# KlrShaK/opencv-SimpleSLAM

Measured on AMD Instinct MI355X. Metric: frames/sec ALIKED+LightGlue @1241x376, higher is better.
Workload: dtype f32 (contractions: f16 hi/lo split operands, f32 accumulate; 3 MFMA per product, 2 in attention's P.V = precision 'f16x3p1', the default since r05: profiles/r05_flip_soak.md, r06_flip_soak.md); 1 GPU; C2/C4: synthetic 1241x376x3 uint8 frame stream, ALIKED-n16 extract + LightGlue match (t-1,t), 2048 kpts/frame, min_conf 0.7, random-init weights; inputs resident in HBM before the timed region, features and matches left on the device (the `pcie` leg times the same pipeline with per-round H2D of the frames and D2H of {count, pairs}); max_kpts=2048, lightglue_layers_executed=9, pairs_per_lightglue_launch=8, frames_per_aliked_launch=8

## Files before the change

### opencv-simpleslam_amd/csrc/lg_plan.hpp

```cpp
#pragma once

namespace sslam {

constexpr int LG_NH = 4;
constexpr int LG_NL = 9;
constexpr int LG_AQ = 128;
constexpr int LG_AK = 64;

constexpr int lg_ks_max(int Kc) { return Kc >= 1024 ? 4 : (Kc >= 512 ? 2 : 1); }

struct LGHooks {
    int precision = 2;
    bool sim_exact = false;
    int layers = LG_NL;
    bool self_only = false;
    int key_split = 0;
    int big_gemm = -1;
    int study = 0;
    bool share_frames = true;
};

enum class LGAttn { F32, FourWave, Asm };
enum class LGMerge { None, Launch, InFfn };
enum class LGLinears { Ring, Big };
enum class LGFfnTile { T64, T32 };

struct LGPlan {
    bool split;
    bool proj_split;
    LGAttn attn;
    bool p_single;
    int ks;
    LGMerge merge;
    LGLinears linears;
    LGFfnTile ffn_tile;
    bool heads_in_ffn;
    int layers;
    bool self_only_last;
    bool share_frames;
};

inline LGPlan lg_plan(const LGHooks& h, int Kc, int NI, bool want_heads) {
    LGPlan p{};
    p.split = h.precision != 0;
    p.proj_split = p.split && !h.sim_exact;
    p.layers = h.layers;
    p.self_only_last = h.self_only;
    p.share_frames = h.share_frames && p.split;

    const int k = h.key_split;
    const bool forced = k > 0, by_size = k == 0 || k == -4 || k == -5;
    const bool asm_kernel = k == 0 || k == -3 || k == -5 || k > 100;
    const bool fold_allowed = k == 0 || k > 100;
    p.ks = forced ? (k > 100 ? k - 100 : k) : 1;
    if (by_size) {
        const int units = NI * LG_NH * (Kc / LG_AQ);
        while (p.ks < 4 && units * p.ks < 256 && Kc / LG_AK >= 2 * p.ks * 4) p.ks *= 2;
    }
    if (p.ks > lg_ks_max(Kc)) p.ks = lg_ks_max(Kc);

    if (!p.split) {
        p.attn = LGAttn::F32;
        p.merge = LGMerge::Launch;
        return p;
    }
    p.attn = asm_kernel && !(h.study & 0x04) ? LGAttn::Asm : LGAttn::FourWave;
    p.p_single = h.precision == 2 || (h.study & 0x04);

    const int b = h.big_gemm;
    const bool big = b >= 0 ? b != 0 : ((long)NI * Kc >= 4096 && Kc % 128 == 0);
    p.linears = big ? LGLinears::Big : LGLinears::Ring;
    p.ffn_tile = b == 3 || (b != 2 && NI * (Kc / 64) <= 128) ? LGFfnTile::T32 : LGFfnTile::T64;
    p.heads_in_ffn = big && b != 5 && want_heads;

    if (p.ks == 1) p.merge = LGMerge::None;
    else p.merge = big && p.ffn_tile == LGFfnTile::T32 && h.study == 0 && fold_allowed ? LGMerge::InFfn : LGMerge::Launch;
    return p;
}

template <class PX, class PD, class PC>
inline int lg_alias(int NI, const PX* xy, const PD* desc, const PC* cnt, const int* bound, const float* size_w,
                    const float* size_h, int* rep) {
    int distinct = 0;
    for (int j = 0; j < NI; ++j) {
        rep[j] = j;
        for (int i = 0; i < j; ++i)
            if (xy[i] == xy[j] && desc[i] == desc[j] && cnt[i] == cnt[j] && bound[i] == bound[j] && size_w[i] == size_w[j] &&
                size_h[i] == size_h[j]) {
                rep[j] = i;
                break;
            }
        distinct += rep[j] == j;
    }
    return distinct;
}

}
```

### opencv-simpleslam_amd/csrc/lightglue_kernels.hip

```cpp
#include <mutex>
#include <type_traits>
#include "common.hpp"
#include "gemm_f32.hpp"
#include "gemm_f16x3.hpp"
#include "gemm_f16x3_big.hpp"
#include "ffn_fused.hpp"
#include "lg_plan.hpp"

namespace {

using sslam::f32x16;
using sslam::mfma32;
using sslam::acc_row;
using sslam::GemmSmem;
using sslam::GemmA;
using sslam::gemm_mainloop;
using sslam::half8;
using sslam::half4;
using sslam::SplitPtr;
using sslam::GemmSmemH;
using sslam::GemmAH;
using sslam::gemm_mainloop_h;
using sslam::gemm_mainloop_ring;
using sslam::panel_index;
using sslam::mfma16;
using sslam::split_f32;
using sslam::SPLIT_INV;
using sslam::LGHooks; using sslam::LGPlan; using sslam::LGAttn; using sslam::LGMerge; using sslam::LGLinears; using sslam::LGFfnTile;

constexpr int D = 256;
constexpr int DH = 64;
constexpr int NH = sslam::LG_NH;
constexpr int DIN = 128;
constexpr int NL = sslam::LG_NL;
constexpr int ENC = 32;

struct LGCtrl {
    int n[2];
    int n_prev[2];
// ... 933 lines not shown
    const int img = blockIdx.y, r = p.al.rep[img];
    const LGCtrl& pc = ctrl_of(p.ctrl, img);
    if (pc.stop) return;
    if (blockIdx.x == 0 && threadIdx.x == 0 && *range_flag_of(p.shadow, r)) *range_flag_of(p.ctrl, img) = 1;
    if (r == img) return;
    const unsigned n = (unsigned)pc.n[img & 1];
    const unsigned t = blockIdx.x * blockDim.x + threadIdx.x, nt = gridDim.x * blockDim.x;
    auto copy_rows = [&](void* base, size_t per) {
        uint4* d = reinterpret_cast<uint4*>(base) + (size_t)img * p.Kc * per;
        const uint4* s = reinterpret_cast<const uint4*>(base) + (size_t)r * p.Kc * per;
        for (unsigned u = t; u < n * per; u += nt) d[u] = s[u];
    };
    copy_rows(p.x, D * 4 / 16);
    copy_rows(p.enc_cos, ENC * 4 / 16);
    copy_rows(p.enc_sin, ENC * 4 / 16);
    constexpr unsigned PU = sslam::PANEL_K * 2 / 16;
    const unsigned run = n * PU;
    uint4* hi = reinterpret_cast<uint4*>(p.xs_hi);
    uint4* lo = reinterpret_cast<uint4*>(p.xs_lo);
    for (unsigned u = t; u < run * (D / sslam::PANEL_K); u += nt) {
        const unsigned k = u / run, e = u - k * run;
        const size_t po = (size_t)k * p.rows_total * PU + e;
        const size_t di = po + (size_t)img * p.Kc * PU, si = po + (size_t)r * p.Kc * PU;
        hi[di] = hi[si];
        lo[di] = lo[si];
    }
}

enum { EPH_QKV = 0, EPH_CROSS = 1, EPH_SPLIT = 2, EPH_F32 = 3, EPH_RESID = 4 };

struct LinearArgsH {
    SplitPtr A0, A1; int lda; int K0; int K;
    SplitPtr W; const float* bias; int N;
    float* out; int ldo;
    SplitOut outs;
    SplitOut q, k, vt;
    float q_scale, k_scale;
    const float* enc_cos; const float* enc_sin;
    const LGCtrl* ctrl; int Kc; int NIc;
};

constexpr int RING_MAX = 2;
template <int BM, int BN>
constexpr int ring_depth() {
    constexpr int stage_bytes = sslam::ring_stage_halves<BM, BN>() * 2;
    constexpr int d = (160 * 1024) / stage_bytes;
    return d > RING_MAX ? RING_MAX : (d < 2 ? 2 : d);
}

__device__ __forceinline__ float erf_as(float x) {
    const float ax = fabsf(x);
    const float t = __builtin_amdgcn_rcpf(fmaf(0.3275911f, ax, 1.0f));
    float p = fmaf(t, 1.061405429f, -1.453152027f);
    p = fmaf(p, t, 1.421413741f);
    p = fmaf(p, t, -0.284496736f);
    p = fmaf(p, t, 0.254829592f);
    const float e = __builtin_amdgcn_exp2f(-ax * ax * 1.4426950408889634f);
    return copysignf(fmaf(-p * t, e, 1.0f), x);
}

template <int BM, int BN, int TM, int TN, int WN, int NT, int EPI>
__device__ __forceinline__ void linear_h_epilogue(const LinearArgsH& p, const RowDom& rd, int col0, size_t ibase,
                                                  const f32x16 (&c1)[TM][TN], const f32x16 (&c2)[TM][TN],
                                                  _Float16* lds) {
    const int t = threadIdx.x, lane = t & 63, wave = t >> 6;
    const int wm = wave / WN, wn = wave % WN;
// ... 136 lines not shown
    RowDom rd;
    rd.img = rb / nb; rd.row0 = (rb % nb) * BM; rd.n = n_of(p.ctrl, rd.img);
    if (ctrl_of(p.ctrl, rd.img).stop) return;
    if (rd.row0 >= rd.n) return;
    const int col0 = cb * BN;
    const size_t ibase = (size_t)rd.img * p.Kc;
    GemmAH ga{{p.A0.hi, p.A0.lo}, {p.A1.hi ? p.A1.hi : p.A0.hi, p.A1.lo ? p.A1.lo : p.A0.lo}, p.lda, p.K0};
    f32x16 c1[TM][TN], c2[TM][TN];
    gemm_mainloop_ring<BM, BN, TM, TN, ring_depth<BM, BN>()>(ga, p.W, p.NIc * p.Kc, p.K, (int)ibase + rd.row0,
                                                             (int)ibase + p.Kc, col0, p.N, lg_ring, c1, c2);
    if (threadIdx.x >= 256) return;
    linear_h_epilogue<BM, BN, TM, TN, 2, 256, EPI>(p, rd, col0, ibase, c1, c2, lg_ring);
}

template <int BM, int BN, int WM, int WN, int EPI>
__global__ __launch_bounds__(WM * WN * 64, 2) void lg_linear_big_kernel(LinearArgsH p) {
    extern __shared__ __attribute__((aligned(16))) _Float16 lg_ring[];
    constexpr int TM = BM / (32 * WM), TN = BN / (32 * WN);
    int rb, cb;
    xcd_tile(gridDim.x, rb, cb);
    const int nb = (p.Kc + BM - 1) / BM;
    RowDom rd;
    rd.img = rb / nb; rd.row0 = (rb % nb) * BM; rd.n = n_of(p.ctrl, rd.img);
    if (ctrl_of(p.ctrl, rd.img).stop) return;
    if (rd.row0 >= rd.n) return;
    const int col0 = cb * BN;
    const size_t ibase = (size_t)rd.img * p.Kc;
    GemmAH ga{{p.A0.hi, p.A0.lo}, {p.A1.hi ? p.A1.hi : p.A0.hi, p.A1.lo ? p.A1.lo : p.A0.lo}, p.lda, p.K0};
    f32x16 c1[TM][TN], c2[TM][TN];
    constexpr int NW = WM * WN;
    sslam::gemm_mainloop_big<BM, BN, WM, WN>(ga, p.W, p.NIc * p.Kc, p.K, (int)ibase + rd.row0, (int)ibase + p.Kc, col0,
                                             p.N, lg_ring, c1, c2);
    linear_h_epilogue<BM, BN, TM, TN, WN, NW * 64, EPI>(p, rd, col0, ibase, c1, c2, lg_ring);
}

struct ProjBigArgs {
    const _Float16 *a_hi, *a_lo; int a_rows; int K;
    const _Float16 *w_hi, *w_lo; long w_layer_stride;
    const float* bias; long b_layer_stride; int by_stop_layer; int ignore_stop;
    float out_scale; float* out;
    _Float16 *o_hi, *o_lo; int o_rows;
    const LGCtrl* ctrl; int Kc;
};
template <int BM, int BN, int WM, int WN>
__global__ __launch_bounds__(WM * WN * 64, 2) void lg_proj_big_kernel(ProjBigArgs p) {
    extern __shared__ __attribute__((aligned(16))) _Float16 lg_ring[];
    constexpr int TM = BM / (32 * WM), TN = BN / (32 * WN);
    const int img = blockIdx.z;
    const LGCtrl& pc = ctrl_of(p.ctrl, img);
    if (pc.stop == 2 || (pc.stop && !p.ignore_stop)) return;
    const int n = pc.n[img & 1], row0 = blockIdx.y * BM, col0 = blockIdx.x * BN;
    if (row0 >= n) return;
    const size_t lw = p.by_stop_layer ? (size_t)pc.stop_layer * p.w_layer_stride : 0;
    const float* bias = p.bias + (p.by_stop_layer ? (size_t)pc.stop_layer * p.b_layer_stride : 0);
    const int g0 = img * p.Kc;
    const sslam::SplitPtr a{p.a_hi, p.a_lo};
    GemmAH ga{a, a, 0, p.K};
    f32x16 c1[TM][TN], c2[TM][TN];
    sslam::gemm_mainloop_big<BM, BN, WM, WN>(ga, sslam::SplitPtr{p.w_hi + lw, p.w_lo + lw}, p.a_rows, p.K, g0 + row0, g0 + p.Kc, col0, D,
                                             lg_ring, c1, c2);
    const int lane = threadIdx.x & 63, wave = threadIdx.x >> 6, wm = wave / WN, wn = wave % WN;
    float amax = 0.0f;
    const bool odd = lane & 1;
#pragma unroll
    for (int i = 0; i < TM; ++i)
#pragma unroll
// ... 67 lines not shown
template <int TT, bool FOLD = false>
__global__ __launch_bounds__(512, 2) void lg_ffn_fused_kernel(FfnKArgs p) {
    extern __shared__ __attribute__((aligned(16))) _Float16 lg_ring[];
    constexpr int TOK = 32 * TT;
    const int nb = p.Kc / TOK;
    const int img = blockIdx.x / nb, row0 = (blockIdx.x % nb) * TOK;
    const LGCtrl& pc = ctrl_of(p.ctrl, img);
    if (pc.stop) return;
    const int n = pc.n[img & 1];
    if (row0 >= n) return;
    const int ibase = img * p.Kc;
    sslam::FfnFusedArgs f = p.f;
    f.unconf = &const_cast<LGCtrl*>(p.ctrl)[img >> 1].unconf;
    if constexpr (FOLD) { f.part_base = (long)img * NH * p.Kc + row0; f.part_kc = p.Kc; }
    sslam::ffn_fused_tile<TT, FOLD>(f, ibase + row0, ibase + p.Kc, min(TOK, n - row0), range_flag_of(p.ctrl, img), lg_ring);
}


__global__ void lg_pack_ffn_kernel(const float* __restrict__ w1, const float* __restrict__ w2, _Float16* __restrict__ w1f,
                                   _Float16* __restrict__ w2f, int* __restrict__ range_flag) {
    const int i = blockIdx.x * blockDim.x + threadIdx.x;
    if (i < 512 * 512) {
        _Float16 a, b;
        split_f32(w1[i], a, b, range_flag);
        w1f[sslam::ffn_w1_frag_index(0, i >> 9, i & 511)] = a;
        w1f[sslam::ffn_w1_frag_index(1, i >> 9, i & 511)] = b;
    }
    if (i < 256 * 512) {
        _Float16 a, b;
        split_f32(w2[i], a, b, range_flag);
        w2f[sslam::ffn_w2_frag_index(0, i >> 9, i & 511)] = a;
        w2f[sslam::ffn_w2_frag_index(1, i >> 9, i & 511)] = b;
    }
}

__global__ __launch_bounds__(256) void lg_ln_gelu_h_kernel(const float* __restrict__ hid, SplitOut outs,
                                                           const float* __restrict__ gamma,
                                                           const float* __restrict__ beta,
                                                           const LGCtrl* __restrict__ ctrl, int Kc, int NI, int NIc) {
    const int lane = threadIdx.x & 63;
    const int gw = blockIdx.x * 4 + (threadIdx.x >> 6);
    const int img = gw / Kc, row = gw % Kc;
    if (img >= NI || ctrl_of(ctrl, img).stop || row >= n_of(ctrl, img)) return;
    const size_t base = ((size_t)img * Kc + row) * 512;
    const float4 a = *reinterpret_cast<const float4*>(hid + base + lane * 4);
    const float4 b = *reinterpret_cast<const float4*>(hid + base + 256 + lane * 4);
    const float4 ga = *reinterpret_cast<const float4*>(gamma + lane * 4), gb = *reinterpret_cast<const float4*>(gamma + 256 + lane * 4);
    const float4 ba = *reinterpret_cast<const float4*>(beta + lane * 4), bb = *reinterpret_cast<const float4*>(beta + 256 + lane * 4);
    float s = (a.x + a.y) + (a.z + a.w) + (b.x + b.y) + (b.z + b.w);
    for (int o = 32; o > 0; o >>= 1) s += __shfl_xor(s, o);
    const float mean = s / 512.0f;
    float v[8] = {a.x - mean, a.y - mean, a.z - mean, a.w - mean, b.x - mean, b.y - mean, b.z - mean, b.w - mean};
    const float gm[8] = {ga.x, ga.y, ga.z, ga.w, gb.x, gb.y, gb.z, gb.w};
    const float bt[8] = {ba.x, ba.y, ba.z, ba.w, bb.x, bb.y, bb.z, bb.w};
    float q = 0.0f;
#pragma unroll
    for (int i = 0; i < 8; ++i) q += v[i] * v[i];
    for (int o = 32; o > 0; o >>= 1) q += __shfl_xor(q, o);
    const float rstd = 1.0f / sqrtf(q / 512.0f + 1e-5f);
    half4 h0, l0, h1, l1;
#pragma unroll
    for (int i = 0; i < 8; ++i) {
        const float y = v[i] * rstd * gm[i] + bt[i];
        const float g = 0.5f * y * (1.0f + erf_as(y * 0.70710678118654752440f));
        _Float16 hh, ll;
        split_f32(g, hh, ll, range_flag_of(ctrl, img));
// ... 324 lines not shown
struct sslam_lightglue {
    sslam_ctx* ctx = nullptr;
    int Kc = 0;
    int NB = 1;
    int NIc = 2;
    int KSmax = 4;
    float depth_conf = 0.95f, width_conf = 0.99f, filter_thr = 0.1f;
    int prune_min = -1;
    sslam::OwnedSlab slab;
    float* blob = nullptr;
    const float *w_in, *b_in, *w_r;
    LGLayerW L[NL];
    const float *fp_w, *fp_b, *mt_w, *mt_b;
    long fp_stride = 0, mt_stride = 0;
    const float* tc_w[NL - 1];
    const float* tc_b[NL - 1];
    LGCtrl* ctrl;
    LGCtrl* ctrl_shadow;
    int last_distinct = 0;
    bool last_fanout = false;
    int* range_sticky;
    float *x, *enc_cos, *enc_sin, *q, *k, *v, *msg, *hid, *tx, *tc, *ts;
    float *o_part, *m_part, *l_part, *conf, *mat, *md, *sim, *rmax, *rlog, *cmax, *clog, *best0;
    float *cpmax, *cpsum, *cpval, *bbox;
    int* cparg;
    int *ind, *gmap, *prune, *arg0, *arg1;
    float *in_xy, *in_desc, *up_xy, *up_desc, *out_score;
    int32_t *out_ij, *out_info;
    LGHooks hooks;
    hipError_t launch_error = hipSuccess;
    _Float16* zero_plane = nullptr;
    _Float16 *w_hi, *w_lo;
    _Float16 *ffn_w1f[NL][2], *ffn_w2f[NL][2];
    _Float16 *xs_hi, *xs_lo, *msgs_hi, *msgs_lo, *hids_hi, *hids_lo;
    _Float16 *qs_hi, *qs_lo, *ks_hi, *ks_lo, *vts_hi, *vts_lo;
    size_t n_blob = 0;
    bool profile = false;
    std::vector<hipEvent_t> ev;
    size_t ev_used = 0;
    int last_pairs = 1;
    bool use_graphs = false;
    sslam::GraphCache graphs;
    void settings_changed() { if (!graphs.entries.empty()) { (void)hipStreamSynchronize(ctx->stream); graphs.clear(); } }
    ~sslam_lightglue() {
        for (hipEvent_t e : ev) (void)hipEventDestroy(e);
        if (zero_plane) (void)hipFree(zero_plane);
    }
};

namespace {

size_t pad64(size_t n) { return (n + 63) / 64 * 64; }

int lg_bind_weights(sslam_lightglue* g, size_t n_floats) {
    size_t off = 0;
    auto take = [&](size_t n) { const float* p = g->blob + off; off += pad64(n); return p; };
    g->w_in = take((size_t)D * DIN); g->b_in = take(D); g->w_r = take(ENC * 2);
    for (int i = 0; i < NL; ++i) {
        LGLayerW& l = g->L[i];
        l.wqkv = take(3 * D * D); l.bqkv = take(3 * D);
        l.w1 = take(4 * D * D); l.b1 = take(2 * D); l.lnw = take(2 * D); l.lnb = take(2 * D);
        l.w2 = take(2 * D * D); l.b2 = take(D);
        l.cqkv = take(2 * D * D); l.cbqkv = take(2 * D);
        l.cw1 = take(4 * D * D); l.cb1 = take(2 * D); l.clnw = take(2 * D); l.clnb = take(2 * D);
        l.cw2 = take(2 * D * D); l.cb2 = take(D);
    }
// ... 65 lines not shown
}

void launch_ffn(sslam_lightglue* g, hipStream_t s, int NI, const float* message, const float* w1,
                const float* b1, const float* lnw, const float* lnb, const float* w2, const float* b2) {
    LinearArgs a = lin(g, NI, g->x, D, message, D, D, 2 * D, w1, b1, 2 * D);
    a.out = g->hid; a.ldo = 2 * D;
    launch_linear<64, 128, 1, 2, EPI_PLAIN>(s, a);
    hipLaunchKernelGGL(lg_ln_gelu_kernel, dim3(sslam::cdiv(NI * g->Kc, 4)), dim3(256), 0, s, g->hid, lnw,
                       lnb, g->ctrl, g->Kc, NI);
    LinearArgs c = lin(g, NI, g->hid, 2 * D, nullptr, 0, 2 * D, 2 * D, w2, b2, D);
    c.out = g->x; c.ldo = D;
    launch_linear<64, 64, 1, 1, EPI_RESID>(s, c);
}

SplitPtr wsp(const sslam_lightglue* g, const float* w) {
    const size_t off = (size_t)(w - g->blob);
    return SplitPtr{g->w_hi + off, g->w_lo + off};
}

template <int BM, int BN, int WM, int WN, int EPI>
void launch_linear_big(hipStream_t s, int NI, const LinearArgsH& a) {
    constexpr int NW = WM * WN;
    constexpr size_t stage = (size_t)sslam::BIG_STAGES * sslam::big_stage_halves<BM, BN>() * sizeof(_Float16);
    constexpr size_t epi = (size_t)BM * (BN + 4) * sizeof(float);
    constexpr size_t lds = stage > epi ? stage : epi;
    static_assert(lds <= 160 * 1024, "LDS budget");
    if (!a.ctrl) {
        (void)hipFuncSetAttribute((const void*)lg_linear_big_kernel<BM, BN, WM, WN, EPI>,
                                  hipFuncAttributeMaxDynamicSharedMemorySize, (int)lds);
        return;
    }
    dim3 grid(a.N / BN, NI * sslam::cdiv(a.Kc, BM));
    hipLaunchKernelGGL((lg_linear_big_kernel<BM, BN, WM, WN, EPI>), grid, dim3(NW * 64), lds, s, a);
}

template <int BM, int BN, int TM, int TN, int EPI>
void launch_linear_h(hipStream_t s, int NI, const LinearArgsH& a) {
    constexpr size_t lds = (size_t)ring_depth<BM, BN>() * sslam::ring_stage_halves<BM, BN>() * sizeof(_Float16);
    if (!a.ctrl) {
        (void)hipFuncSetAttribute((const void*)lg_linear_h_kernel<BM, BN, TM, TN, EPI>,
                                  hipFuncAttributeMaxDynamicSharedMemorySize, (int)lds);
        return;
    }
    dim3 grid(a.N / BN, NI * sslam::cdiv(a.Kc, BM));
    hipLaunchKernelGGL((lg_linear_h_kernel<BM, BN, TM, TN, EPI>), grid, dim3(512), lds, s, a);
}

LinearArgsH linh(const sslam_lightglue* g, const LGCtrl* ctrl, SplitPtr A0, SplitPtr A1, int lda, int K0, int K, const float* W,
                 const float* b, int N) {
    LinearArgsH a{};
    a.A0 = A0; a.A1 = A1; a.lda = lda; a.K0 = K0; a.K = K;
    a.W = wsp(g, W); a.bias = b; a.N = N; a.ctrl = ctrl; a.Kc = g->Kc; a.NIc = g->NIc;
    a.enc_cos = g->enc_cos; a.enc_sin = g->enc_sin; a.q_scale = 1.0f; a.k_scale = 1.0f;
    return a;
}

extern "C" const unsigned char sslam_lg_attention_asm_hsaco[];
extern "C" const unsigned char sslam_lg_attention_asm_p1_hsaco[];
struct AttnAsmArgs {
    const _Float16 *q_hi, *q_lo, *k_hi, *k_lo, *vt_hi, *vt_lo;
    _Float16 *msg_hi, *msg_lo;
    const LGCtrl* ctrl;
    int cross, Kc, NIc, nqb, nslab;
    unsigned magic;
    int nih, lks;
    float *o_part, *m_part, *l_part;
// ... 72 lines not shown
            if (cross && heads) {
                const bool do_stop = g->depth_conf > 0.0f;
                k.f.hm = g->mt_w + (size_t)layer * g->mt_stride; k.f.hm_b = g->mt_b + (size_t)layer * g->mt_stride;
                k.f.hc = do_stop ? g->tc_w[layer] : nullptr; k.f.hc_b = do_stop ? g->tc_b[layer] : nullptr;
                k.f.conf_thr = conf_threshold(layer); k.f.conf = g->conf; k.f.mat = g->mat;
            }
            k.ctrl = ctrl; k.Kc = g->Kc;
            if (plan.merge == LGMerge::InFfn) {
                k.f.o_part = g->o_part; k.f.m_part = g->m_part; k.f.l_part = g->l_part;
                k.f.ks = plan.ks; k.f.part_zs = (long)g->NIc * NH * g->Kc;
                hipLaunchKernelGGL((lg_ffn_fused_kernel<1, true>), dim3(NI * (g->Kc / 32)), dim3(512), sslam::FFN_LDS_BYTES, s, k);
            } else if (plan.ffn_tile == LGFfnTile::T32)
                hipLaunchKernelGGL(lg_ffn_fused_kernel<1>, dim3(NI * (g->Kc / 32)), dim3(512), sslam::FFN_LDS_BYTES, s, k);
            else
                hipLaunchKernelGGL(lg_ffn_fused_kernel<2>, dim3(NI * (g->Kc / 64)), dim3(512), sslam::FFN_LDS_BYTES, s, k);
            return;
        }
        LinearArgsH a = linh(g, ctrl, act(xs, 0x20), act(msgs, 0x20), D, D, 2 * D, w1, b1, 2 * D);
        wgt(a, 0x80);
        a.out = g->hid; a.ldo = 2 * D;
        launch_linear_h<64, 128, 1, 2, EPH_F32>(s, NI, a);
        hipLaunchKernelGGL(lg_ln_gelu_h_kernel, dim3(tokblocks), dim3(256), 0, s, g->hid,
                           SplitOut{g->hids_hi, g->hids_lo}, lnw, lnb, ctrl, g->Kc, NI, g->NIc);
        LinearArgsH c = linh(g, ctrl, act(hids, 0x20), none, 2 * D, 2 * D, 2 * D, w2, b2, D);
        wgt(c, 0x80);
        c.out = g->x; c.ldo = D; c.outs = SplitOut{g->xs_hi, g->xs_lo};
        launch_linear_h<64, 64, 1, 1, EPH_RESID>(s, NI, c);
    };
    {
        LinearArgsH a = linh(g, self_ctrl, act(xs, 0x10), none, D, D, D, l.wqkv, l.bqkv, 3 * D);
        wgt(a, 0x40);
        a.q = SplitOut{g->qs_hi, g->qs_lo}; a.k = SplitOut{g->ks_hi, g->ks_lo}; a.vt = SplitOut{g->vts_hi, g->vts_lo};
        a.q_scale = sm_scale; a.k_scale = 1.0f;
        if (big) launch_linear_big<128, 128, 2, 2, EPH_QKV>(s, NI, a);
        else launch_linear_h<64, 192, 1, 3, EPH_QKV>(s, NI, a);
    }
    launch_attention_h(g, s, plan, NI, self_ctrl, qs, ks, vts, 0);
    ffn(0, self_ctrl, l.w1, l.b1, l.lnw, l.lnb, l.w2, l.b2);
    if (shared) {
        const FanoutArgs a{g->x, g->enc_cos, g->enc_sin, g->xs_hi, g->xs_lo, g->Kc, g->NIc * g->Kc, g->ctrl, g->ctrl_shadow, *shared};
        hipLaunchKernelGGL(lg_fanout_kernel, dim3(FANOUT_BLOCKS_PER_IMAGE, NI), dim3(256), 0, s, a);
    }
    if (self_only) return;
    {
        LinearArgsH a = linh(g, g->ctrl, act(xs, 0x10), none, D, D, D, l.cqkv, l.cbqkv, 2 * D);
        wgt(a, 0x40);
        a.q = SplitOut{g->qs_hi, g->qs_lo}; a.vt = SplitOut{g->vts_hi, g->vts_lo};
        a.q_scale = sqrtf(sm_scale);
        if (big) launch_linear_big<128, 128, 2, 2, EPH_CROSS>(s, NI, a);
        else launch_linear_h<64, 128, 1, 2, EPH_CROSS>(s, NI, a);
    }
    launch_attention_h(g, s, plan, NI, g->ctrl, qs, qs, vts, 1);
    ffn(1, g->ctrl, l.cw1, l.cb1, l.clnw, l.clnb, l.cw2, l.cb2);
}

AliasTab lg_alias_table(const LGPlan& plan, const StageSrc& src, int NI, bool& shared) {
    AliasTab al{};
    int rep[2 * MAX_PAIRS];
    al.distinct = sslam::lg_alias(NI, src.xy, src.desc, src.cnt, src.bound, src.size_w, src.size_h, rep);
    shared = plan.share_frames && al.distinct < NI;
    for (int i = 0; i < 2 * MAX_PAIRS; ++i) al.rep[i] = (signed char)(shared && i < NI ? rep[i] : i);
    return al;
}

int lg_enqueue(sslam_lightglue* g, int pairs, const StageSrc& src, float min_conf, int32_t* ij_out,
               float* score_out, int32_t* info_out, long out_stride) {
    hipStream_t s = g->ctx->stream;
    (void)hipGetLastError();
    const int Kc = g->Kc, NI = 2 * pairs;
    const LGPlan plan = sslam::lg_plan(g->hooks, Kc, NI, g->depth_conf > 0.0f || g->width_conf > 0.0f);
    bool shared = false;
    const AliasTab al = lg_alias_table(plan, src, NI, shared);
    const LGCtrl* const c0 = shared ? g->ctrl_shadow : g->ctrl;
    hipLaunchKernelGGL(lg_prepare_kernel, dim3(NI, 8), dim3(1024), 0, s, src, Kc, g->in_xy, g->in_desc, g->bbox,
                       g->ind, g->prune, g->ctrl, al, shared ? g->ctrl_shadow : nullptr);
    hipLaunchKernelGGL(lg_posenc_kernel, dim3(sslam::cdiv(NI * Kc * ENC, 256)), dim3(256), 0, s, g->in_xy,
                       g->bbox, g->w_r, g->enc_cos, g->enc_sin, Kc, NI, c0);
    const bool proj_h = plan.proj_split;
    constexpr size_t big_lds = (size_t)sslam::BIG_STAGES * sslam::big_stage_halves<128, 128>() * sizeof(_Float16);
    const dim3 biggrid(D / 128, sslam::cdiv(Kc, 128), NI);
    if (proj_h) {
        hipLaunchKernelGGL(lg_split_rows_kernel, dim3(SPLIT_BLOCKS_PER_IMAGE, NI), dim3(256), 0, s, g->in_desc, g->ks_hi, g->ks_lo, DIN, Kc,
// ... 86 lines not shown
        dim3 grid(sslam::cdiv(Kc, 128), sslam::cdiv(Kc, 64), pairs);
        hipLaunchKernelGGL((lg_sim_kernel<64, 128, 1, 2>), grid, dim3(256), 0, s, a);
    }
    hipLaunchKernelGGL(lg_row_stats_kernel, dim3(sslam::cdiv(Kc, 4), pairs), dim3(256), 0, s, g->sim, g->rmax,
                       g->rlog, Kc, g->ctrl);
    hipLaunchKernelGGL(lg_col_stats_kernel, dim3(sslam::cdiv(Kc, 64), CSLAB, pairs), dim3(256), 0, s, g->sim,
                       g->cpmax, g->cpsum, Kc, g->ctrl);
    hipLaunchKernelGGL(lg_col_stats_merge_kernel, dim3(sslam::cdiv(Kc, 256), pairs), dim3(256), 0, s, g->cpmax,
                       g->cpsum, g->cmax, g->clog, Kc, g->ctrl);
    hipLaunchKernelGGL(lg_col_argmax_kernel, dim3(sslam::cdiv(Kc, 64), CSLAB, pairs), dim3(256), 0, s, g->sim,
                       g->rmax, g->rlog, g->cmax, g->clog, g->conf, g->cpval, g->cparg, Kc, g->ctrl);
    hipLaunchKernelGGL(lg_row_argmax_kernel, dim3(sslam::cdiv(Kc, 4), pairs), dim3(256), 0, s, g->sim, g->rmax,
                       g->rlog, g->cmax, g->clog, g->conf, g->best0, g->arg0, g->cpval, g->cparg, g->arg1, Kc, g->ctrl);
    hipLaunchKernelGGL(lg_emit_kernel, dim3(pairs), dim3(1024), 0, s, g->best0, g->arg0, g->arg1, g->ind,
                       g->filter_thr, min_conf, ij_out, score_out, info_out, g->ctrl, Kc, out_stride, g->range_sticky);
    SSLAM_HIP_CHECK(hipGetLastError());
    if (g->launch_error != hipSuccess) {
        const hipError_t e = g->launch_error;
        g->launch_error = hipSuccess;
        SSLAM_HIP_CHECK(e);
    }
    return 0;
}

void lg_configure_kernels() {
    static bool done = false;
    if (done) return;
    done = true;
    const LinearArgsH cfg{};
    hipStream_t s = nullptr;
    launch_linear_h<64, 128, 1, 2, EPH_F32>(s, 0, cfg);   launch_linear_h<64, 64, 1, 1, EPH_RESID>(s, 0, cfg);
    launch_linear_h<64, 192, 1, 3, EPH_QKV>(s, 0, cfg);   launch_linear_h<64, 128, 1, 2, EPH_CROSS>(s, 0, cfg);
    launch_linear_big<128, 128, 2, 2, EPH_QKV>(s, 0, cfg); launch_linear_big<128, 128, 2, 2, EPH_CROSS>(s, 0, cfg);
    {
        constexpr int big_lds = sslam::BIG_STAGES * sslam::big_stage_halves<128, 128>() * (int)sizeof(_Float16);
        (void)hipFuncSetAttribute((const void*)lg_proj_big_kernel<128, 128, 2, 2>, hipFuncAttributeMaxDynamicSharedMemorySize, big_lds);
        (void)hipFuncSetAttribute((const void*)lg_sim_big_kernel<128, 128, 2, 2>, hipFuncAttributeMaxDynamicSharedMemorySize, big_lds);
    }
    (void)hipFuncSetAttribute((const void*)lg_ffn_fused_kernel<1>, hipFuncAttributeMaxDynamicSharedMemorySize, sslam::FFN_LDS_BYTES);
    (void)hipFuncSetAttribute((const void*)lg_ffn_fused_kernel<1, true>, hipFuncAttributeMaxDynamicSharedMemorySize, sslam::FFN_LDS_BYTES);
    (void)hipFuncSetAttribute((const void*)lg_ffn_fused_kernel<2>, hipFuncAttributeMaxDynamicSharedMemorySize, sslam::FFN_LDS_BYTES);
}

void lg_note_sharing(sslam_lightglue* g, int pairs, const StageSrc& src) {
    const LGPlan plan = sslam::lg_plan(g->hooks, g->Kc, 2 * pairs, g->depth_conf > 0.0f || g->width_conf > 0.0f);
    g->last_distinct = lg_alias_table(plan, src, 2 * pairs, g->last_fanout).distinct;
}

int lg_enqueue_cached(sslam_lightglue* g, int pairs, const StageSrc& src, float min_conf, int32_t* ij_out,
                      float* score_out, int32_t* info_out, long out_stride) {
    g->last_pairs = pairs;
    lg_note_sharing(g, pairs, src);
    if (!g->use_graphs || g->profile)
        return lg_enqueue(g, pairs, src, min_conf, ij_out, score_out, info_out, out_stride);
    std::vector<uint64_t> key{(uint64_t)pairs, (uint64_t)ij_out, (uint64_t)score_out, (uint64_t)info_out,
                              (uint64_t)out_stride, 0};
    memcpy(&key[5], &min_conf, sizeof(float));
    for (int i = 0; i < 2 * pairs; ++i) {
        key.push_back((uint64_t)src.xy[i]); key.push_back((uint64_t)src.desc[i]);
        key.push_back((uint64_t)src.cnt[i]); key.push_back((uint64_t)src.bound[i]);
        uint64_t sz = 0; memcpy(&sz, &src.size_w[i], 4); memcpy((char*)&sz + 4, &src.size_h[i], 4);
        key.push_back(sz);
    }
    return sslam::run_cached(g->graphs, g->ctx->stream, key, [&] {
        return lg_enqueue(g, pairs, src, min_conf, ij_out, score_out, info_out, out_stride);
    });
// ... 20 lines not shown
    g->NB = max_pairs; g->NIc = 2 * max_pairs;
    g->KSmax = sslam::lg_ks_max(Kc);
    if (const char* e = getenv("SSLAM_LG_SIM_EXACT")) g->hooks.sim_exact = e[0] == '1';
    const size_t K = (size_t)Kc, NI = (size_t)g->NIc, NB = (size_t)max_pairs;
    auto bind = [&](sslam::Slab& A) {
        g->blob = A.take<float>(n_floats);
        g->ctrl = A.take<LGCtrl>(NB); g->ctrl_shadow = A.take<LGCtrl>(NB);
        g->range_sticky = A.take<int>(4);
        g->x = A.take<float>(NI * K * D); g->msg = A.take<float>(NI * K * D);
        g->tx = A.take<float>(NI * K * D); g->md = A.take<float>(NI * K * D);
        g->hid = A.take<float>(NI * K * 2 * D);
        g->q = A.take<float>(NI * K * D); g->k = A.take<float>(NI * K * D); g->v = A.take<float>(NI * K * D);
        g->enc_cos = A.take<float>(NI * K * ENC); g->enc_sin = A.take<float>(NI * K * ENC);
        g->tc = A.take<float>(NI * K * ENC); g->ts = A.take<float>(NI * K * ENC);
        g->o_part = A.take<float>((size_t)g->KSmax * NI * NH * K * DH);
        g->m_part = A.take<float>((size_t)g->KSmax * NI * NH * K);
        g->l_part = A.take<float>((size_t)g->KSmax * NI * NH * K);
        g->conf = A.take<float>(NI * K); g->mat = A.take<float>(NI * K); g->bbox = A.take<float>(NI * 4);
        g->sim = A.take<float>(NB * K * K);
        g->rmax = A.take<float>(NB * K); g->rlog = A.take<float>(NB * K); g->cmax = A.take<float>(NB * K);
        g->clog = A.take<float>(NB * K); g->best0 = A.take<float>(NB * K);
        g->ind = A.take<int>(NI * K); g->gmap = A.take<int>(NI * K); g->prune = A.take<int>(NI * K);
        g->arg0 = A.take<int>(NB * K); g->arg1 = A.take<int>(NB * K);
        g->cpmax = A.take<float>(NB * CSLAB * K); g->cpsum = A.take<float>(NB * CSLAB * K);
        g->cpval = A.take<float>(NB * CSLAB * K); g->cparg = A.take<int>(NB * CSLAB * K);
        g->in_xy = A.take<float>(NI * K * 2); g->in_desc = A.take<float>(NI * K * DIN);
        g->up_xy = A.take<float>(2 * K * 2); g->up_desc = A.take<float>(2 * K * DIN);
        g->out_ij = A.take<int32_t>(2 * K); g->out_score = A.take<float>(K); g->out_info = A.take<int32_t>(8);
        g->w_hi = A.take<_Float16>(n_floats); g->w_lo = A.take<_Float16>(n_floats);
        for (int i = 0; i < NL; ++i)
            for (int c = 0; c < 2; ++c) {
                g->ffn_w1f[i][c] = A.take<_Float16>((size_t)2 * 4 * D * D);
                g->ffn_w2f[i][c] = A.take<_Float16>((size_t)2 * 2 * D * D);
            }
        g->xs_hi = A.take<_Float16>(NI * K * D); g->xs_lo = A.take<_Float16>(NI * K * D);
        g->msgs_hi = A.take<_Float16>(NI * K * D); g->msgs_lo = A.take<_Float16>(NI * K * D);
        g->hids_hi = A.take<_Float16>(NI * K * 2 * D); g->hids_lo = A.take<_Float16>(NI * K * 2 * D);
        g->qs_hi = A.take<_Float16>(NI * K * D); g->qs_lo = A.take<_Float16>(NI * K * D);
        g->ks_hi = A.take<_Float16>(NI * K * D); g->ks_lo = A.take<_Float16>(NI * K * D);
        g->vts_hi = A.take<_Float16>(NI * K * D); g->vts_lo = A.take<_Float16>(NI * K * D);
    };
    if (int rc = g->slab.alloc("sslam_lightglue_create", true, bind)) return rc;
    SSLAM_HIP_CHECK(hipMemcpy(g->blob, weights, n_floats * 4, hipMemcpyHostToDevice));
    if (int rc = lg_bind_weights(g.get(), n_floats)) return rc;
    g->n_blob = n_floats;
    {
        auto splitw = [&](const float* w, int N, int K) {
            const size_t off = (size_t)(w - g->blob), n = (size_t)N * K;
            hipLaunchKernelGGL(lg_split_weight_kernel, dim3((unsigned)((n + 255) / 256)), dim3(256), 0, ctx->stream,
                               w, g->w_hi + off, g->w_lo + off, N, K, g->range_sticky);
        };
        for (int i = 0; i < NL; ++i) {
            const LGLayerW& l = g->L[i];
            splitw(l.wqkv, 3 * D, D); splitw(l.w1, 2 * D, 2 * D); splitw(l.w2, D, 2 * D);
            splitw(l.cqkv, 2 * D, D); splitw(l.cw1, 2 * D, 2 * D); splitw(l.cw2, D, 2 * D);
            hipLaunchKernelGGL(lg_pack_ffn_kernel, dim3(4 * D * D / 256), dim3(256), 0, ctx->stream, l.w1, l.w2,
                               g->ffn_w1f[i][0], g->ffn_w2f[i][0], g->range_sticky);
            hipLaunchKernelGGL(lg_pack_ffn_kernel, dim3(4 * D * D / 256), dim3(256), 0, ctx->stream, l.cw1, l.cw2,
                               g->ffn_w1f[i][1], g->ffn_w2f[i][1], g->range_sticky);
        }
        splitw(g->w_in, D, DIN);
        for (int i = 0; i < NL; ++i) splitw(g->fp_w + (size_t)i * g->fp_stride, D, D);
        int wflag = 0;
        if (int rc = lg_take_range_flag(g.get(), &wflag)) return rc;
        SSLAM_REQUIRE(!wflag, "sslam_lightglue_create: a weight with |value| >= 65520 does not fit the fp16 planes of the "
                              "split-precision path");
    }
    sslam::ctx_retain(ctx);
    *out = g.release();
    return 0;
}

int sslam_lightglue_create(sslam_ctx* ctx, const float* weights, size_t n_floats, int max_kpts,
                           sslam_lightglue** out) {
    return sslam_lightglue_create_batched(ctx, weights, n_floats, max_kpts, 1, out);
}

int sslam_lightglue_destroy(sslam_lightglue* g) {
    return sslam::destroy_instance(g);
}

int sslam_lightglue_set_conf(sslam_lightglue* g, float depth_confidence, float width_confidence,
                             float filter_threshold, int prune_min_kpts) {
    SSLAM_REQUIRE(g != nullptr, "sslam_lightglue_set_conf: NULL instance");
    g->settings_changed();
    g->depth_conf = depth_confidence; g->width_conf = width_confidence;
    g->filter_thr = filter_threshold; g->prune_min = prune_min_kpts;
    return 0;
}

int sslam_lightglue_match_batch_dev(sslam_lightglue* g, int n_pairs, const float* const* xy0,
                                    const float* const* desc0, const int32_t* const* m_dev, const int32_t* M,
// ... 137 lines not shown
    }
    *total_ms_out = tot;
    *launches_out = (int32_t)(g->ev_used / 2);
    g->ev_used = 0;
    return 0;
}

int sslam_lightglue_set_precision(sslam_lightglue* g, int mode) {
    SSLAM_REQUIRE(g != nullptr && (mode == 0 || mode == 1 || mode == 2), "sslam_lightglue_set_precision: bad argument");
    g->settings_changed();
    g->hooks.precision = mode;
    return 0;
}

int sslam_lightglue_debug_layers(sslam_lightglue* g, int layers, int self_only) {
    SSLAM_REQUIRE(g != nullptr && layers >= 1 && layers <= NL, "sslam_lightglue_debug_layers: bad argument");
    g->settings_changed();
    g->hooks.layers = layers; g->hooks.self_only = self_only != 0;
    return 0;
}

int sslam_lightglue_debug_key_split(sslam_lightglue* g, int ks) {
    SSLAM_REQUIRE(g != nullptr && ((ks >= -5 && ks <= 2 && ks != -2) || ks == 4 || ks == 101 || ks == 102 || ks == 104),
                  "sslam_lightglue_debug_key_split: ks must be -5 (split by size, assembly kernel, the merge as a launch of its own), "
                  "-4 (split by size, r02 4-wave kernel), -3 (no split, assembly kernel), "
                  "-1 (no split, r02 4-wave kernel), 0, 1, 2 or 4 (forced split, r02 4-wave kernel), 101, 102 or 104 (forced split, "
                  "assembly kernel)");
    g->settings_changed();
    g->hooks.key_split = ks;
    return 0;
}

int sslam_lightglue_debug_big_gemm(sslam_lightglue* g, int mode) {
    SSLAM_REQUIRE(g != nullptr && mode >= -1 && mode <= 5 && mode != 4, "sslam_lightglue_debug_big_gemm: bad argument");
    g->settings_changed();
    g->hooks.big_gemm = mode;
    return 0;
}

int sslam_lightglue_debug_split_form(sslam_lightglue* g, int mask) {
    SSLAM_REQUIRE(g != nullptr && mask >= 0 && mask <= 0xff, "sslam_lightglue_debug_split_form: bad argument");
    g->settings_changed();
    if (mask && !g->zero_plane) {
        const size_t act = (size_t)g->NIc * g->Kc * 2 * D, wmax = (size_t)4 * D * D;
        const size_t n = (act > wmax ? act : wmax) * sizeof(_Float16);
        SSLAM_HIP_CHECK(hipSetDevice(g->ctx->device));
        SSLAM_HIP_CHECK(hipMalloc((void**)&g->zero_plane, n));
        SSLAM_HIP_CHECK(hipMemset(g->zero_plane, 0, n));
    }
    g->hooks.study = mask;
    return 0;
}

int sslam_lightglue_debug_share_frames(sslam_lightglue* g, int enable) {
    SSLAM_REQUIRE(g != nullptr && (enable == 0 || enable == 1), "sslam_lightglue_debug_share_frames: bad argument");
    g->settings_changed();
    g->hooks.share_frames = enable != 0;
    return 0;
}

int sslam_lightglue_debug_share_info(sslam_lightglue* g, int32_t* out) {
    SSLAM_REQUIRE(g && out, "sslam_lightglue_debug_share_info: NULL argument");
    out[0] = g->last_distinct; out[1] = g->last_fanout ? 1 : 0;
    return 0;
}

int sslam_lightglue_use_graphs(sslam_lightglue* g, int enable) {
// ... 25 lines not shown
```

Measured before the change: 1256 frames/s.

## Add resident-activation projection kernel with prepacked fragment-ordered QKV weights

Adds a projection kernel for the self QKV and cross QK/V linears. Each block loads a 64-token hi/lo activation tile into LDS once and sweeps every output column block, streaming weights prepacked into MFMA fragment order straight into registers through an 8-deep register ring. It is meant to cut repeated activation reloads and the LDS staging of weights that the tiled big GEMM pays for. The cost is extra weight storage and pack kernels at creation, plus fewer, longer-running blocks per launch, which may leave the GPU underfilled when token counts are small.

```diff
diff --git a/opencv-simpleslam_amd/csrc/lg_plan.hpp b/opencv-simpleslam_amd/csrc/lg_plan.hpp
--- a/opencv-simpleslam_amd/csrc/lg_plan.hpp
+++ b/opencv-simpleslam_amd/csrc/lg_plan.hpp
@@ -33,6 +33,7 @@
     int ks;
     LGMerge merge;
     LGLinears linears;
+    bool proj_resident;
     LGFfnTile ffn_tile;
     bool heads_in_ffn;
     int layers;
@@ -70,6 +71,7 @@
     const int b = h.big_gemm;
     const bool big = b >= 0 ? b != 0 : ((long)NI * Kc >= 4096 && Kc % 128 == 0);
     p.linears = big ? LGLinears::Big : LGLinears::Ring;
+    p.proj_resident = big && b != 6 && h.study == 0;
     p.ffn_tile = b == 3 || (b != 2 && NI * (Kc / 64) <= 128) ? LGFfnTile::T32 : LGFfnTile::T64;
     p.heads_in_ffn = big && b != 5 && want_heads;
 
diff --git a/opencv-simpleslam_amd/csrc/lightglue_kernels.hip b/opencv-simpleslam_amd/csrc/lightglue_kernels.hip
--- a/opencv-simpleslam_amd/csrc/lightglue_kernels.hip
+++ b/opencv-simpleslam_amd/csrc/lightglue_kernels.hip
@@ -5,6 +5,7 @@
 #include "gemm_f16x3.hpp"
 #include "gemm_f16x3_big.hpp"
 #include "ffn_fused.hpp"
+#include "proj_resident.hpp"
 #include "lg_plan.hpp"
 
 namespace {
@@ -1004,6 +1005,7 @@
 struct LinearArgsH {
     SplitPtr A0, A1; int lda; int K0; int K;
     SplitPtr W; const float* bias; int N;
+    const _Float16* wf;
     float* out; int ldo;
     SplitOut outs;
     SplitOut q, k, vt;
@@ -1206,6 +1208,24 @@
     sslam::gemm_mainloop_big<BM, BN, WM, WN>(ga, p.W, p.NIc * p.Kc, p.K, (int)ibase + rd.row0, (int)ibase + p.Kc, col0,
                                              p.N, lg_ring, c1, c2);
     linear_h_epilogue<BM, BN, TM, TN, WN, NW * 64, EPI>(p, rd, col0, ibase, c1, c2, lg_ring);
+}
+
+template <int EPI>
+__global__ __launch_bounds__(512, 2) void lg_linear_resident_kernel(LinearArgsH p) {
+    extern __shared__ __attribute__((aligned(16))) _Float16 lg_ring[];
+    static_assert(EPI == EPH_QKV || EPI == EPH_CROSS, "the two projections of a block");
+    constexpr int NB = (EPI == EPH_QKV ? 3 : 2) * D / sslam::PR_BN;
+    const int nb = p.Kc / sslam::PR_TOK;
+    RowDom rd;
+    rd.img = blockIdx.x / nb; rd.row0 = (blockIdx.x % nb) * sslam::PR_TOK; rd.n = n_of(p.ctrl, rd.img);
+    if (ctrl_of(p.ctrl, rd.img).stop) return;
+    if (rd.row0 >= rd.n) return;
+    const size_t ibase = (size_t)rd.img * p.Kc;
+    _Float16* const stage = lg_ring + sslam::PR_TILE_BYTES / 2;
+    sslam::proj_resident_tile<NB>(p.A0, p.NIc * p.Kc, p.wf, (int)ibase + rd.row0, (int)ibase + p.Kc, lg_ring,
+                                  [&](int cb, const f32x16 (&c1)[2][1], const f32x16 (&c2)[2][1]) {
+        linear_h_epilogue<sslam::PR_TOK, sslam::PR_BN, 2, 1, 8, 512, EPI>(p, rd, cb * sslam::PR_BN, ibase, c1, c2, stage);
+    });
 }
 
 struct ProjBigArgs {
@@ -1339,6 +1359,15 @@
         w2f[sslam::ffn_w2_frag_index(0, i >> 9, i & 511)] = a;
         w2f[sslam::ffn_w2_frag_index(1, i >> 9, i & 511)] = b;
     }
+}
+
+__global__ void lg_pack_proj_kernel(const float* __restrict__ w, int N, _Float16* __restrict__ wf, int* __restrict__ range_flag) {
+    const int i = blockIdx.x * blockDim.x + threadIdx.x;
+    if (i >= N * D) return;
+    _Float16 a, b;
+    split_f32(w[i], a, b, range_flag);
+    wf[sslam::proj_w_frag_index(0, i / D, i % D)] = a;
+    wf[sslam::proj_w_frag_index(1, i / D, i % D)] = b;
 }
 
 __global__ __launch_bounds__(256) void lg_ln_gelu_h_kernel(const float* __restrict__ hid, SplitOut outs,
@@ -1729,6 +1758,7 @@
     _Float16* zero_plane = nullptr;
     _Float16 *w_hi, *w_lo;
     _Float16 *ffn_w1f[NL][2], *ffn_w2f[NL][2];
+    _Float16* proj_wf[NL][2];
     _Float16 *xs_hi, *xs_lo, *msgs_hi, *msgs_lo, *hids_hi, *hids_lo;
     _Float16 *qs_hi, *qs_lo, *ks_hi, *ks_lo, *vts_hi, *vts_lo;
     size_t n_blob = 0;
@@ -1860,6 +1890,16 @@
     }
     dim3 grid(a.N / BN, NI * sslam::cdiv(a.Kc, BM));
     hipLaunchKernelGGL((lg_linear_big_kernel<BM, BN, WM, WN, EPI>), grid, dim3(NW * 64), lds, s, a);
+}
+
+template <int EPI>
+void launch_linear_resident(hipStream_t s, int NI, const LinearArgsH& a) {
+    if (!a.ctrl) {
+        (void)hipFuncSetAttribute((const void*)lg_linear_resident_kernel<EPI>, hipFuncAttributeMaxDynamicSharedMemorySize,
+                                  sslam::PR_LDS_BYTES);
+        return;
+    }
+    hipLaunchKernelGGL(lg_linear_resident_kernel<EPI>, dim3(NI * (a.Kc / sslam::PR_TOK)), dim3(512), sslam::PR_LDS_BYTES, s, a);
 }
 
 template <int BM, int BN, int TM, int TN, int EPI>
@@ -1998,7 +2038,9 @@
         wgt(a, 0x40);
         a.q = SplitOut{g->qs_hi, g->qs_lo}; a.k = SplitOut{g->ks_hi, g->ks_lo}; a.vt = SplitOut{g->vts_hi, g->vts_lo};
         a.q_scale = sm_scale; a.k_scale = 1.0f;
-        if (big) launch_linear_big<128, 128, 2, 2, EPH_QKV>(s, NI, a);
+        a.wf = g->proj_wf[layer][0];
+        if (plan.proj_resident) launch_linear_resident<EPH_QKV>(s, NI, a);
+        else if (big) launch_linear_big<128, 128, 2, 2, EPH_QKV>(s, NI, a);
         else launch_linear_h<64, 192, 1, 3, EPH_QKV>(s, NI, a);
     }
     launch_attention_h(g, s, plan, NI, self_ctrl, qs, ks, vts, 0);
@@ -2013,7 +2055,9 @@
         wgt(a, 0x40);
         a.q = SplitOut{g->qs_hi, g->qs_lo}; a.vt = SplitOut{g->vts_hi, g->vts_lo};
         a.q_scale = sqrtf(sm_scale);
-        if (big) launch_linear_big<128, 128, 2, 2, EPH_CROSS>(s, NI, a);
+        a.wf = g->proj_wf[layer][1];
+        if (plan.proj_resident) launch_linear_resident<EPH_CROSS>(s, NI, a);
+        else if (big) launch_linear_big<128, 128, 2, 2, EPH_CROSS>(s, NI, a);
         else launch_linear_h<64, 128, 1, 2, EPH_CROSS>(s, NI, a);
     }
     launch_attention_h(g, s, plan, NI, g->ctrl, qs, qs, vts, 1);
@@ -2166,6 +2210,7 @@
     launch_linear_h<64, 128, 1, 2, EPH_F32>(s, 0, cfg);   launch_linear_h<64, 64, 1, 1, EPH_RESID>(s, 0, cfg);
     launch_linear_h<64, 192, 1, 3, EPH_QKV>(s, 0, cfg);   launch_linear_h<64, 128, 1, 2, EPH_CROSS>(s, 0, cfg);
     launch_linear_big<128, 128, 2, 2, EPH_QKV>(s, 0, cfg); launch_linear_big<128, 128, 2, 2, EPH_CROSS>(s, 0, cfg);
+    launch_linear_resident<EPH_QKV>(s, 0, cfg);            launch_linear_resident<EPH_CROSS>(s, 0, cfg);
     {
         constexpr int big_lds = sslam::BIG_STAGES * sslam::big_stage_halves<128, 128>() * (int)sizeof(_Float16);
         (void)hipFuncSetAttribute((const void*)lg_proj_big_kernel<128, 128, 2, 2>, hipFuncAttributeMaxDynamicSharedMemorySize, big_lds);
@@ -2252,6 +2297,7 @@
             for (int c = 0; c < 2; ++c) {
                 g->ffn_w1f[i][c] = A.take<_Float16>((size_t)2 * 4 * D * D);
                 g->ffn_w2f[i][c] = A.take<_Float16>((size_t)2 * 2 * D * D);
+                g->proj_wf[i][c] = A.take<_Float16>((size_t)2 * (c ? 2 : 3) * D * D);
             }
         g->xs_hi = A.take<_Float16>(NI * K * D); g->xs_lo = A.take<_Float16>(NI * K * D);
         g->msgs_hi = A.take<_Float16>(NI * K * D); g->msgs_lo = A.take<_Float16>(NI * K * D);
@@ -2278,6 +2324,10 @@
                                g->ffn_w1f[i][0], g->ffn_w2f[i][0], g->range_sticky);
             hipLaunchKernelGGL(lg_pack_ffn_kernel, dim3(4 * D * D / 256), dim3(256), 0, ctx->stream, l.cw1, l.cw2,
                                g->ffn_w1f[i][1], g->ffn_w2f[i][1], g->range_sticky);
+            hipLaunchKernelGGL(lg_pack_proj_kernel, dim3(3 * D * D / 256), dim3(256), 0, ctx->stream, l.wqkv, 3 * D,
+                               g->proj_wf[i][0], g->range_sticky);
+            hipLaunchKernelGGL(lg_pack_proj_kernel, dim3(2 * D * D / 256), dim3(256), 0, ctx->stream, l.cqkv, 2 * D,
+                               g->proj_wf[i][1], g->range_sticky);
         }
         splitw(g->w_in, D, DIN);
         for (int i = 0; i < NL; ++i) splitw(g->fp_w + (size_t)i * g->fp_stride, D, D);
@@ -2481,7 +2531,7 @@
 }
 
 int sslam_lightglue_debug_big_gemm(sslam_lightglue* g, int mode) {
-    SSLAM_REQUIRE(g != nullptr && mode >= -1 && mode <= 5 && mode != 4, "sslam_lightglue_debug_big_gemm: bad argument");
+    SSLAM_REQUIRE(g != nullptr && mode >= -1 && mode <= 6 && mode != 4, "sslam_lightglue_debug_big_gemm: bad argument");
     g->settings_changed();
     g->hooks.big_gemm = mode;
     return 0;
diff --git a/opencv-simpleslam_amd/csrc/proj_resident.hpp b/opencv-simpleslam_amd/csrc/proj_resident.hpp
--- /dev/null
+++ b/opencv-simpleslam_amd/csrc/proj_resident.hpp
@@ -0,0 +1,118 @@
+#pragma once
+#include "ffn_fused.hpp"
+
+namespace sslam {
+
+constexpr int PR_TOK = 64;
+constexpr int PR_K = 256;
+constexpr int PR_BN = 256;
+constexpr int PR_STEPS = PR_K / 16;
+constexpr int PR_DEPTH = 8;
+constexpr int PR_CHUNKS = PR_K / (2 * PANEL_K);
+constexpr int PR_TILE_BYTES = 2 * PR_TOK * PR_K * 2;
+constexpr int PR_STAGE_BYTES = PR_TOK * (PR_BN + 4) * 4;
+constexpr int PR_LDS_BYTES = PR_TILE_BYTES + PR_STAGE_BYTES;
+static_assert(PR_STEPS % PR_DEPTH == 0 && PR_DEPTH % 2 == 0, "the ring of fragment sets divides a block's steps, even depth");
+
+__host__ __device__ inline size_t proj_w_frag_index(int plane, int n, int k) {
+    const int cb = n >> 8, w = (n >> 5) & 7, lr = n & 31, ks = k >> 4, h = (k >> 3) & 1, e = k & 7;
+    return (((((size_t)cb * PR_STEPS + ks) * 8 + w) * 2 + plane) * 64 + (h * 32 + lr)) * 8 + e;
+}
+
+constexpr int proj_ops_after_chunk(int c) {
+    return c == 0 ? 2 * (PR_DEPTH - 1) + 2 * (PR_CHUNKS - 1) : 2 * (PR_CHUNKS - 1 - c) + 2 * (4 * c - 1);
+}
+
+template <int NB, class Epi>
+__device__ __forceinline__ void proj_resident_tile(SplitPtr xs, int plane_rows, const _Float16* wf, int grow0, int grow_cap,
+                                                   _Float16* smem, Epi&& epilogue) {
+    const int t = threadIdx.x, lane = t & 63;
+    const int wave = __builtin_amdgcn_readfirstlane(t >> 6);
+    const int h = lane >> 5, lr = lane & 31;
+    const int lane16 = lane * 16;
+
+    const auto r_w = ffn_rsrc(wf, (unsigned)NB * 2 * PR_BN * PR_K * 2);
+    auto load_w = [&](int g, half8 (&dst)[2]) {
+        const int base = (g * 8 + wave) * 2048;
+        dst[0] = ffn_ldfrag(r_w, lane16, base);
+        dst[1] = ffn_ldfrag(r_w, lane16, base + 1024);
+    };
+
+    half8 wq[PR_DEPTH][2];
+    load_w(0, wq[0]);
+    const int prow = lane >> 2, pc = lane & 3;
+    const int psw = (pc ^ ((prow >> 2) & 3)) * 8;
+    const int aoff = (min(grow0 + (wave & 3) * 16 + prow, grow_cap - 1) * PANEL_K + psw) * 2;
+    const bool lo = wave >= 4;
+    const auto r_a = ffn_rsrc(lo ? xs.lo : xs.hi, (unsigned)plane_rows * PR_K * 2);
+    const int pstride = plane_rows * (PANEL_K * 2);
+    auto issue_chunk = [&](int c) {
+#pragma unroll
+        for (int j = 0; j < 2; ++j) {
+            const int kp = 2 * c + j;
+            ffn_dma16(r_a, aoff, kp * pstride, smem + ((kp * 2 + (lo ? 1 : 0)) * 64 + (wave & 3) * 16) * 32);
+        }
+    };
+    issue_chunk(0);
+    __builtin_amdgcn_sched_barrier(0);
+#pragma unroll
+    for (int d = 1; d < PR_DEPTH; ++d) load_w(d, wq[d]);
+#pragma unroll
+    for (int c = 1; c < PR_CHUNKS; ++c) issue_chunk(c);
+    __builtin_amdgcn_sched_barrier(0);
+    ffn_wait_vm<proj_ops_after_chunk(0)>();
+    __builtin_amdgcn_s_barrier();
+
+    const int fsw = (lr >> 2) & 3;
+    auto read_a = [&](int ks, half8 (&ah)[2], half8 (&al)[2]) {
+        const int kp = ks >> 1, s = ks & 1;
+        const _Float16* base = smem + (kp * 2 * 64 + lr) * 32 + (((2 * s + h) ^ fsw) * 8);
+#pragma unroll
+        for (int tt = 0; tt < 2; ++tt) {
+            ah[tt] = *reinterpret_cast<const half8*>(base + tt * 32 * 32);
+            al[tt] = *reinterpret_cast<const half8*>(base + 64 * 32 + tt * 32 * 32);
+        }
+    };
+
+#pragma unroll 1
+    for (int cb = 0; cb < NB; ++cb) {
+        f32x16 acc1[2][1], acc2[2][1];
+#pragma unroll
+        for (int tt = 0; tt < 2; ++tt)
+#pragma unroll
+            for (int r = 0; r < 16; ++r) { acc1[tt][0][r] = 0.0f; acc2[tt][0][r] = 0.0f; }
+        auto mma = [&](const half8 (&w)[2], const half8 (&ah)[2], const half8 (&al)[2]) {
+#pragma unroll
+            for (int tt = 0; tt < 2; ++tt) {
+                acc1[tt][0] = mfma16(ah[tt], w[0], acc1[tt][0]);
+                acc2[tt][0] = mfma16(ah[tt], w[1], acc2[tt][0]);
+                acc2[tt][0] = mfma16(al[tt], w[0], acc2[tt][0]);
+            }
+        };
+        half8 ah0[2], al0[2], ah1[2], al1[2];
+        read_a(0, ah0, al0);
+        ffn_static_for([&](auto ks_c) {
+            constexpr int ks = decltype(ks_c)::value, u = ks % PR_DEPTH;
+            if constexpr (ks % 4 == 3 && ks + 1 < PR_STEPS) {
+                if (cb == 0) {
+                    ffn_wait_vm<proj_ops_after_chunk((ks + 1) / 4)>();
+                    __builtin_amdgcn_s_barrier();
+                }
+            }
+            if constexpr (ks & 1) {
+                if constexpr (ks + 1 < PR_STEPS) read_a(ks + 1, ah0, al0);
+                __builtin_amdgcn_sched_barrier(0);
+                mma(wq[u], ah1, al1);
+            } else {
+                read_a(ks + 1, ah1, al1);
+                __builtin_amdgcn_sched_barrier(0);
+                mma(wq[u], ah0, al0);
+            }
+            load_w(cb * PR_STEPS + ks + PR_DEPTH, wq[u]);
+            __builtin_amdgcn_sched_barrier(0);
+        }, std::make_integer_sequence<int, PR_STEPS>{});
+        epilogue(cb, acc1, acc2);
+    }
+}
+
+}
```

Result: no change. 1264 frames/s (median of 6 runs) (+0.6%).
